# kolomeytsev/EB-CADRL

Measured on AMD Instinct MI355X. Metric: agent-steps/sec, higher is better.
Workload: dtype f64; 1 GPU; metric: 4096 envs/GPU x 10 humans + 8 static rows, ORCA + kinematics + collisions + reward + rotated obs (T=17), one ebc_step (one HIP launch) per step, auto-reset; envs_per_gpu=4096, humans=10, parallelism=env-slice x1

## Files before the change

### eb-cadrl_amd/csrc/ebc_kernels.h

```cpp
#pragma once

#include "ebc_device.h"

#ifndef EBC_ENV_PRIO
#define EBC_ENV_PRIO 3
#endif
#ifndef EBC_ORCA_PRIO
#define EBC_ORCA_PRIO 1
#endif
#ifndef EBC_POLL_SLEEP
#define EBC_POLL_SLEEP 2
#endif
#include "ebc_orca_group.h"
#include "ebc_scene_gen.h"
#include "ebc_step_rules.h"

namespace ebc {

struct DevState {
  int E, N, S, G;
  int *n_humans;
  double *px, *py, *vx, *vy, *gx, *gy, *radius, *v_pref;
  uint8_t *type;
  int *n_static;
  double *spx, *spy, *sradius;
  int *grid_scene;
  double *robot;
  double *robot_n;
  double *time;
  double *arrival;
  uint8_t *done;
  double *hact;
  uint4 *vel;
  unsigned long long *env_done;
  unsigned *rows_loaded;
  unsigned *robot_ready;
  unsigned *fault;
  ScenePool pool;
  float4 *tile;
  float inv_time_horizon, inv_time_step, range_sq;
  unsigned n_magic, n_shift;
};

#ifndef EBC_SPIN_LIMIT
#define EBC_SPIN_LIMIT (1u << 22)
#endif

struct StepIO {
  const double *robot_action;
  double border[4];
  int has_border;
  int robot_policy;
  int auto_reset;
  double *reward;
  uint8_t *done;
  uint8_t *info;
  double *dmin;
  double *dist_to_goal;
  double *robot_action_out;
  double *human_action;
  double *ob;
  float *obs_rotated;
};

struct LookIO {
  const double *actions;
  int A;
  double border[4];
  int has_border;
  double *reward;
  uint8_t *done;
  uint8_t *info;
  double *dmin;
  double *next_ob;
  float *rows;
};

__device__ __forceinline__ void store_tile(const EbcParams &p, const DevState &s, size_t k, double px,
                                           double py, double vx, double vy, double gx, double gy,
                                           double rad, double vpref) {
  float prefx, prefy;
  orca_pref_velocity(px, py, gx, gy, prefx, prefy);
  s.tile[2 * k] = make_float4((float)px, (float)py, (float)vx, (float)vy);
  s.tile[2 * k + 1] = make_float4((float)(rad + 0.01 + p.orca_safety_space), (float)vpref, prefx, prefy);
}

__global__ __launch_bounds__(256) void pool_pref_kernel(DevState s, size_t first, size_t count) {
  const size_t q = (size_t)blockIdx.x * blockDim.x + threadIdx.x;
  if (q >= count) return;
  const size_t k = first + q;
  float prefx, prefy;
  orca_pref_velocity(s.pool.px[k], s.pool.py[k], s.pool.gx[k], s.pool.gy[k], prefx, prefy);
  s.pool.pref[k] = make_float2(prefx, prefy);
}

__global__ __launch_bounds__(256) void rehome_grid_kernel(DevState s, uint64_t *grid) {
  const int e = blockIdx.x;
// ... 178 lines not shown
  const float posx = (float)rb[0], posy = (float)rb[1], velx = (float)rb[2], vely = (float)rb[3];
  float radius = (float)(rb[4] + 0.01 + safety_space), maxSpeed = (float)rb[7];
  float prefx, prefy;
  orca_pref_velocity(rb[0], rb[1], rb[5], rb[6], prefx, prefy);
  float opx = 0, opy = 0, ovx = 0, ovy = 0, orad = 0;
  if (valid) {
    opx = (float)row.px;
    opy = (float)row.py;
    ovx = (float)row.vx;
    ovy = (float)row.vy;
    orad = (float)(row.radius + 0.01 + safety_space);
  }
  if (sim.rows && l.e_ok) {
    const bool rebuild = sim.rows[ee] != n + ns;
    const size_t q = ee * (size_t)(N + S) + j;
    if (rebuild) {
      if (valid) sim.radius[q] = orad;
      if (j == 0) {
        sim.self[ee] = make_float2(radius, maxSpeed);
        sim.rows[ee] = n + ns;
      }
    } else {
      if (valid) orad = sim.radius[q];
      const float2 me = sim.self[ee];
      radius = me.x;
      maxSpeed = me.y;
    }
  }
  before_solve();
  orca_group<GS>(p, j, group, valid, posx, posy, velx, vely, radius, maxSpeed, prefx, prefy, opx, opy, ovx, ovy,
                 orad, dist_lds + group * L::Sh::DIST, lines_lds + group * L::Sh::LINES,
                 segs_lds + group * L::Sh::LINES, proj_lds + group * L::Sh::LINES, N + S, s.range_sq,
                 s.inv_time_horizon, s.inv_time_step, ox, oy);
}

template <int GS>
__global__ __launch_bounds__(EBC_WAVE) void orca_robot_kernel(EbcParams p, DevState s, double safety_space, double *act, RobotSim sim) {
  __shared__ __align__(16) unsigned char scratch[OrcaLds<GS>::BYTES];
  const RobotLane l = robot_lane<GS>(s);
  const ObsRow row = obs_row(env_rows(s, l.ee), l.j, l.n, l.ns);
  float ox, oy;
  orca_robot_solve<GS>(p, s, safety_space, sim, scratch, l, s.robot + l.ee * 9, row, ox, oy);
  if (l.e_ok && l.j == 0) {
    act[2 * l.ee] = (double)ox;
    act[2 * l.ee + 1] = (double)oy;
  }
}

template <typename Tp>
__device__ __forceinline__ void pin(Tp &x) {
  asm volatile("" : "+v"(x));
}

template <typename Tp>
__device__ __forceinline__ const Tp &read_late(const Tp &x) {
  typedef const Tp __attribute__((address_space(3))) *LdsPtr;
  unsigned off = (unsigned)(size_t)(LdsPtr)&x;
  asm volatile("" : "+v"(off));
  return *(const Tp *)(LdsPtr)(size_t)off;
}

struct ArgBlock {
  EbcParams p;
  DevState s;
  StepIO io;
};
template <typename Tp>
__device__ __forceinline__ void stage_args(Tp *dst_lds, const Tp &src, int lane) {
  const uint32_t *from = reinterpret_cast<const uint32_t *>(&src);
  uint32_t *to = reinterpret_cast<uint32_t *>(dst_lds);
  for (int w = lane; w < (int)(sizeof(Tp) / 4); w += EBC_WAVE) to[w] = from[w];
}

struct LaneMap {
  int el, i, n, ns;
  size_t ee, k;
  bool env_ok, active, leader;
};
struct HumanRegs {
  double px, py, vx, vy, gx, gy, rad, vpref, arrival;
  int type;
};

__device__ __forceinline__ LaneMap lane_map(const DevState &s, int e0, int epb, int lane) {
  LaneMap m;
  const int N = s.N;
  m.el = lane / N;
  m.i = lane - m.el * N;
  const int e = e0 + m.el;
  m.env_ok = m.el < epb && e < s.E;
  m.ee = m.env_ok ? (size_t)e : 0;
  m.k = m.ee * N + m.i;
  m.n = m.env_ok ? s.n_humans[m.ee] : 0;
  m.ns = (m.env_ok && s.S) ? s.n_static[m.ee] : 0;
  m.active = m.env_ok && m.i < m.n;
  m.leader = m.env_ok && m.i == 0;
  return m;
}

__device__ __forceinline__ HumanRegs load_human(const DevState &s, const LaneMap &m) {
  HumanRegs h = {0, 0, 0, 0, 0, 0, 0, 0, 0, 0};
  if (m.env_ok) {
    h.px = s.px[m.k];
    h.py = s.py[m.k];
    h.vx = s.vx[m.k];
    h.vy = s.vy[m.k];
    h.gx = s.gx[m.k];
    h.gy = s.gy[m.k];
    h.rad = s.radius[m.k];
    h.vpref = s.v_pref[m.k];
    h.type = s.type[m.k];
    h.arrival = s.arrival[m.k];
  }
  return h;
}

#define EBC_MAXT 4
struct CommitPre {
  int cursor;
  double sx[EBC_MAXT], sy[EBC_MAXT], sr[EBC_MAXT];
  double px, py, vx, vy, gx, gy, rad, vpref, spx, spy, srad, robot[9];
  int type, n_humans, n_static;
};

template <bool WITH_ROBOT = true>
__device__ __forceinline__ CommitPre preload_commit(const DevState &s, const StepIO &io, const LaneMap &m) {
  CommitPre c;
#pragma unroll
  for (int t = 0; t < EBC_MAXT; ++t) {
    const int r = m.i + t * s.N;
    const bool st = m.env_ok && (io.ob || io.obs_rotated) && r >= m.n && r - m.n < m.ns;
    const size_t q = m.ee * s.S + (st ? r - m.n : 0);
    c.sx[t] = st ? s.spx[q] : 0.0;
    c.sy[t] = st ? s.spy[q] : 0.0;
    c.sr[t] = st ? s.sradius[q] : 0.0;
  }
  c.cursor = 0;
  c.px = c.py = c.vx = c.vy = c.gx = c.gy = c.rad = c.vpref = c.spx = c.spy = c.srad = 0;
  c.type = c.n_humans = c.n_static = 0;
#pragma unroll
  for (int q = 0; q < 9; ++q) c.robot[q] = 0;
  if (io.auto_reset && m.env_ok) {
    const ScenePool &P = s.pool;
    c.cursor = P.P > 0 ? P.cursor[m.ee] : (int)m.ee;
    const size_t src = (size_t)c.cursor * s.N + m.i;
    c.n_humans = P.n_humans[c.cursor];
    c.px = P.px[src]; c.py = P.py[src]; c.vx = P.vx[src]; c.vy = P.vy[src];
    c.gx = P.gx[src]; c.gy = P.gy[src]; c.rad = P.radius[src]; c.vpref = P.v_pref[src];
    c.type = P.type[src];
    if (s.S) {
      c.n_static = P.n_static[c.cursor];
      if (m.i < s.S) {
        const size_t q = (size_t)c.cursor * s.S + m.i;
        c.spx = P.spx[q]; c.spy = P.spy[q]; c.srad = P.sradius[q];
      }
    }
    if (WITH_ROBOT && m.leader) {
#pragma unroll
      for (int q = 0; q < 9; ++q) c.robot[q] = P.robot[(size_t)c.cursor * 9 + q];
    }
  }
  return c;
}

__device__ __forceinline__ void pin_loads(HumanRegs &h, CommitPre &c, double (&rb)[9], double &gtime) {
  pin(h.px); pin(h.py); pin(h.vx); pin(h.vy); pin(h.gx); pin(h.gy); pin(h.rad); pin(h.vpref);
  pin(h.arrival); pin(h.type);
  pin(c.cursor);
#pragma unroll
  for (int q = 0; q < 9; ++q) pin(rb[q]);
#pragma unroll
  for (int t = 0; t < EBC_MAXT; ++t) { pin(c.sx[t]); pin(c.sy[t]); pin(c.sr[t]); }
  pin(gtime);
// ... 288 lines not shown
    h.px = h.px + ax * dt;
    h.py = h.py + ay * dt;
    h.vx = ax;
    h.vy = ay;
    if (h.arrival == 0 && norm2(h.px - h.gx, h.py - h.gy) < h.rad) h.arrival = tnew;
  } else {
    ax = 0;
    ay = 0;
  }
  const RotFrame f = rot_frame(rbn, p.rotate_unicycle);
  pin_pool(pre);
  if (m.leader && !restore) {
#pragma unroll
    for (int c = 0; c < 9; ++c) A.robot[c] = rbn[c];
    *A.time = tnew;
  }
  if (A.human_action) {
    A.human_action[0] = ax;
    A.human_action[1] = ay;
  }
  if (io.ob || io.obs_rotated) {
    int t = 0;
    for (int r = m.i; r < R; r += N, ++t) {
      double opx = 0, opy = 0, ovx = 0, ovy = 0, orad = 0;
      int otype = 0;
      bool valid = false;
      if (r < m.n) {
        opx = h.px; opy = h.py; ovx = h.vx; ovy = h.vy; orad = h.rad; otype = h.type;
        valid = true;
      } else if (r - m.n < m.ns) {
        if (t < EBC_MAXT) {
          opx = t == 0 ? pre.sx[0] : t == 1 ? pre.sx[1] : t == 2 ? pre.sx[2] : pre.sx[3];
          opy = t == 0 ? pre.sy[0] : t == 1 ? pre.sy[1] : t == 2 ? pre.sy[2] : pre.sy[3];
          orad = t == 0 ? pre.sr[0] : t == 1 ? pre.sr[1] : t == 2 ? pre.sr[2] : pre.sr[3];
        } else {
          const size_t q = m.ee * S + (r - m.n);
          opx = s.spx[q]; opy = s.spy[q]; orad = s.sradius[q];
        }
        otype = EBC_ADULT_STATIC;
        valid = true;
      }
      if (A.ob) {
        double *o = A.ob + (size_t)r * 5;
        o[0] = opx; o[1] = opy; o[2] = ovx; o[3] = ovy; o[4] = orad;
      }
      if (A.obs) {
        float out[T];
        if (valid) {
          rotate_row<T>(f, opx, opy, ovx, ovy, orad, otype, out);
        } else {
#pragma unroll
          for (int c = 0; c < T; ++c) out[c] = 0.0f;
        }
        float *o = A.obs + (m.ee * R + r) * T;
#pragma unroll
        for (int c = 0; c < T; ++c) o[c] = out[c];
      }
    }
  }
  commit_state_tail(p, s, m, h, pre, A, restore);
}

__device__ __forceinline__ void load_robot(const DevState &s, const LaneMap &m, double rb[9]) {
  const double *rb_in = s.robot + m.ee * 9;
#pragma unroll
  for (int c = 0; c < 9; ++c) rb[c] = m.env_ok ? rb_in[c] : 0.0;
}

template <int POLICY, int T>
__global__ __launch_bounds__(EBC_WAVE) void step_kernel(EbcParams p_in, DevState s_in, StepIO io_in) {
  const WaveTrace wt(1);
  const int lane = threadIdx.x;
  __shared__ ArgBlock args;
  __shared__ EnvScratch env_scratch;
  __shared__ double sh_rbn[EBC_WAVE][9];
  stage_args(&args.p, p_in, lane);
  stage_args(&args.s, s_in, lane);
  stage_args(&args.io, io_in, lane);
  wave_sync();
  const EbcParams &p = args.p;
  const DevState &s = args.s;
  const StepIO &io = args.io;
  const int epb = EBC_WAVE / s.N;
  const LaneMap m = lane_map(s, blockIdx.x * epb, epb, lane);
  double rb[9];
  load_robot(s, m, rb);
  double gtime = m.env_ok ? s.time[m.ee] : 0.0;
  HumanRegs h = load_human(s, m);
  CommitPre pre = preload_commit(s, io, m);
  const CommitAddr A = commit_addr(s, io, m);
  double ax = 0, ay = 0;
  if (POLICY == EBC_HUMAN_LINEAR) {
    if (m.active) linear_policy(h.px, h.py, h.gx, h.gy, h.vpref, ax, ay);
  } else if (m.env_ok) {
    ax = s.hact[m.k * 2];
    ay = s.hact[m.k * 2 + 1];
  }
  pin_loads(h, pre, rb, gtime);
  pin(ax);
  pin(ay);
  int done_flag = service_env(p, s, io, m, h, rb, gtime, lane, env_scratch);
  if (m.leader) {
#pragma unroll
    for (int c = 0; c < 9; ++c) sh_rbn[m.el][c] = rb[c];
  }
  done_flag = __shfl(done_flag, lane - m.i, EBC_WAVE);
  wave_sync();
  if (!m.env_ok) return;
  double rbn[9];
#pragma unroll
  for (int c = 0; c < 9; ++c) rbn[c] = sh_rbn[m.el][c];
  service_commit<T>(p, s, io, m, h, pre, A, rbn, io.auto_reset && done_flag, gtime + p.time_step, ax, ay);
}

struct StepGrid {
  unsigned env_blocks, orca_blocks, rows_blocks;
  unsigned rows_epw;
  unsigned epoch;
  unsigned total;
};

#define EBC_RBN_ENVS 16
struct RoleLds {
  ArgBlock args;
  union {
    double restart_robot[EBC_RBN_ENVS][9];
    EnvScratch env;
  };
};

#define EBC_ENV_LANES 4
__device__ __forceinline__ void env_lane_role(const EbcParams &p_in, const DevState &s_in, const StepIO &io_in, RoleLds &L,
                                              unsigned block, unsigned epoch, int lane) {
  stage_args(&L.args.p, p_in, lane);
  stage_args(&L.args.s, s_in, lane);
  stage_args(&L.args.io, io_in, lane);
  wave_sync();
  const EbcParams &p = L.args.p;
  const DevState &s = L.args.s;
  const StepIO &io = L.args.io;
  constexpr int Q = EBC_ENV_LANES, EPW = EBC_WAVE / Q;
  const int el = lane / Q, part = lane - el * Q;
  const int e0 = (int)block * EPW;
  const int e = e0 + el;
  const bool ok = e < s.E;
  const size_t ee = ok ? (size_t)e : 0;
  const int N = s.N;
  double rb[9];
#pragma unroll
  for (int c = 0; c < 9; ++c) rb[c] = ok ? s.robot[ee * 9 + c] : 0.0;
  const int n = ok ? s.n_humans[ee] : 0;
  double gtime = ok ? s.time[ee] : 0.0;
  int grid_slot = (ok && s.pool.grid) ? s.grid_scene[ee] : 0;
  const int chunk = (N + Q - 1) / Q;
  const int i0 = part * chunk;
  pin(gtime); pin(grid_slot);
#pragma unroll
  for (int c = 0; c < 9; ++c) pin(rb[c]);
  double a0 = 0, a1 = 0;
  if (ok) robot_action(io.robot_policy, io.robot_action, ee, rb, a0, a1);
  EBC_MARK(1);
  {
    double rn[9];
#pragma unroll
    for (int c = 0; c < 9; ++c) rn[c] = rb[c];
    robot_advance(p, rn, a0, a1);
    double *stage = &L.env.cand[0][0];
    if (part == 0) {
#pragma unroll
      for (int c = 0; c < 9; ++c) stage[el * 9 + c] = rn[c];
      L.env.gtime[el] = gtime;
      L.env.slot[el] = grid_slot;
      L.env.goal[el][0] = rb[5];
      L.env.goal[el][1] = rb[6];
      L.env.ract[el][0] = rn[0];
      L.env.ract[el][1] = rn[1];
    }
    wave_sync();
    const int here = min(EPW, s.E - e0);
    for (int q = lane; q < 9 * here; q += EBC_WAVE)
      __hip_atomic_store(s.robot_n + (size_t)e0 * 9 + q, stage[q], __ATOMIC_RELAXED, __HIP_MEMORY_SCOPE_AGENT);
  }
  constexpr int PRE = 2;
  double hpx[PRE], hpy[PRE], hvx[PRE], hvy[PRE], hr[PRE];
  int ht[PRE];
  {
    const DevState &sl = read_late(s);
#pragma unroll
    for (int q = 0; q < PRE; ++q) {
      const int i = i0 + q;
      const bool have = ok && q < chunk && i < N;
      const size_t k = ee * N + (have ? i : 0);
      hpx[q] = have ? sl.px[k] : 0.0; hpy[q] = have ? sl.py[k] : 0.0; hvx[q] = have ? sl.vx[k] : 0.0; hvy[q] = have ? sl.vy[k] : 0.0;
      hr[q] = have ? sl.radius[k] : 0.0;
      ht[q] = have ? (int)sl.type[k] : 0;
    }
  }
  double rvx, rvy;
  if (p.robot_kinematics == EBC_HOLONOMIC) {
    rvx = a0;
    rvy = a1;
  } else {
    rvx = a0 * cos(a1 + rb[8]);
    rvy = a0 * sin(a1 + rb[8]);
  }
  double dmin[3] = {INFINITY, INFINITY, INFINITY};
  int coll[4] = {0, 0, 0, 0};
  auto visit = [&](double px, double py, double vx, double vy, double r, int t) {
    const double d = closest_dist(px, py, vx, vy, r, rb[0], rb[1], rb[4], rvx, rvy, p.time_step);
#pragma unroll
    for (int q = 0; q < 3; ++q) {
      if (t == q && !coll[q]) {
        if (d < 0) coll[q] = 1;
        else if (d < dmin[q]) dmin[q] = d;
      }
    }
  };
#pragma unroll
  for (int q = 0; q < PRE; ++q)
    if (q < chunk && i0 + q < n) visit(hpx[q], hpy[q], hvx[q], hvy[q], hr[q], ht[q]);
  for (int q = PRE; q < chunk; ++q) {
    const int i = i0 + q;
    if (!__any(i < n)) break;
    if (i < n) {
      const size_t k = ee * N + i;
      visit(s.px[k], s.py[k], s.vx[k], s.vy[k], s.radius[k], (int)s.type[k]);
    }
  }
  asm volatile("s_waitcnt vmcnt(0)" ::: "memory");
  if (ok && part == 0) mailbox_put(s.robot_ready + ee, epoch);
  double fm[3] = {INFINITY, INFINITY, INFINITY};
  int fc[3] = {0, 0, 0};
  const int base = lane - part;
#pragma unroll
  for (int src = 0; src < Q; ++src) {
#pragma unroll
    for (int t = 0; t < 3; ++t) {
      const double od = __shfl(dmin[t], base + src, EBC_WAVE);
      const int oc = __shfl(coll[t], base + src, EBC_WAVE);
      if (!fc[t]) {
        fm[t] = od < fm[t] ? od : fm[t];
        fc[t] = oc;
      }
    }
  }
  EBC_MARK(2);
  if (ok && part == 0) {
    const EnvScratch &XL = read_late(L.env);
    const double nx = XL.ract[el][0], ny = XL.ract[el][1];
    int c4[4] = {fc[0], fc[1], fc[2], 0};
    c4[3] = grid_collision(s.pool.grid ? s.pool.grid + (size_t)XL.slot[el] * s.G * 2 : nullptr, s.G, p.map_size_m,
                           p.map_resolution, nx, ny, rb[4], io.has_border ? io.border : nullptr);
    EBC_MARK(3);
    const RewardOut ro = reward_compute(p, nx, ny, XL.goal[el][0], XL.goal[el][1], rb[4], a1, XL.gtime[el], fm, c4);
    s.done[ee] = (uint8_t)ro.done;
    if (io.reward) io.reward[ee] = ro.reward;
    if (io.done) io.done[ee] = (uint8_t)ro.done;
    if (io.info) io.info[ee] = (uint8_t)ro.info;
    if (io.dmin) {
      io.dmin[3 * ee] = fm[0];
      io.dmin[3 * ee + 1] = fm[1];
      io.dmin[3 * ee + 2] = fm[2];
    }
    if (io.dist_to_goal) io.dist_to_goal[ee] = ro.dist_to_goal;
    if (io.robot_action_out) {
      io.robot_action_out[2 * ee] = a0;
      io.robot_action_out[2 * ee + 1] = a1;
    }
    mailbox_put(s.env_done + ee, ((unsigned long long)epoch << 32) | (1u + (unsigned)ro.done));
  }
  EBC_MARK(4);
}

template <typename Tp>
__device__ __forceinline__ void sreg(const Tp &x) {
  asm volatile("" ::"s"(x));
}

template <int GS>
__device__ __forceinline__ void orca_role(const EbcParams &p, const DevState &s, const OrcaHot &hot, uint4 *vel, unsigned epoch,
                                          unsigned char *scratch, unsigned block, int lane) {
  sreg(s.robot); sreg(s.range_sq); sreg(s.inv_time_horizon); sreg(s.inv_time_step);
  sreg(p.robot_visible); sreg(p.orca_max_neighbors); sreg(p.orca_safety_space);
  constexpr int HPW = EBC_WAVE / GS;
  const int group = lane / GS, j = lane - group * GS;
  const unsigned hh = block * HPW + group;
  const bool h_ok = group < HPW && hh < (unsigned)hot.E * (unsigned)hot.N;
  int e, i;
  split_human(hot, hh, h_ok, e, i);
  float ox, oy;
  bool human_ok;
  orca_wave<GS>(p, s, hot, h_ok, e, i, scratch, ox, oy, human_ok);
#ifdef EBC_WAVE_TRACE
  if (h_ok && (int)hh == g_withhold_human) return;
#endif
  if (h_ok && j == 0) {
    const u32x4 w = {human_ok ? __float_as_uint(ox) : 0u, epoch, human_ok ? __float_as_uint(oy) : 0u, epoch};
    store16_device(vel + hh, w);
  }
}

template <int T>
__device__ __forceinline__ void rows_role(const EbcParams &p_in, const DevState &s_in, const StepIO &io_in,
                                          RoleLds &L, unsigned block, unsigned epw, unsigned epoch, int lane) {
  stage_args(&L.args.p, p_in, lane);
  stage_args(&L.args.s, s_in, lane);
  stage_args(&L.args.io, io_in, lane);
  wave_sync();
  const EbcParams &p = L.args.p;
  const DevState &s = L.args.s;
  const StepIO &io = L.args.io;
  const int N = s.N, S = s.S, R = N + S;
  const int el = R <= EBC_WAVE ? lane / R : 0;
  const int first = lane - el * R;
  const int e = (int)(block * epw) + el;
  const bool env_ok = el < (int)epw && e < s.E;
  const size_t ee = env_ok ? (size_t)e : 0;
  const int stride = R <= EBC_WAVE ? R : EBC_WAVE;
  RotFrame f = {};
  int n = env_ok ? s.n_humans[ee] : 0;
  int ns = (env_ok && S) ? s.n_static[ee] : 0;
  for (int slot = first; slot < R; slot += stride) {
    const bool human = slot < N;
    const size_t k = ee * N + (human ? slot : 0), q = ee * (size_t)(S ? S : 1) + (human ? 0 : slot - N);
    double opx = 0, opy = 0, ovx = 0, ovy = 0, orad = 0;
    int otype = 0;
    if (env_ok && human) {
      opx = s.px[k]; opy = s.py[k]; orad = s.radius[k]; otype = s.type[k];
    } else if (env_ok) {
      opx = s.spx[q]; opy = s.spy[q]; orad = s.sradius[q]; otype = EBC_ADULT_STATIC;
    }
    const uint4 *vbox = s.vel + k;
    pin(opx); pin(opy); pin(orad); pin(otype); pin(vbox); pin(n); pin(ns);
    if (slot == first) {
      mailbox_wait_epoch(s.robot_ready + ee, env_ok, epoch, s.fault);
      double rb[9];
#pragma unroll
      for (int c = 0; c < 9; ++c)
        rb[c] = env_ok ? __hip_atomic_load(s.robot_n + ee * 9 + c, __ATOMIC_RELAXED, __HIP_MEMORY_SCOPE_AGENT) : 0.0;
      f = rot_frame(rb, p.rotate_unicycle);
      pin(f.px); pin(f.py); pin(f.dg);
    }
    if (env_ok && slot + stride >= R && first == 0) mailbox_put(s.rows_loaded + ee, epoch);
    const bool valid = human ? slot < n : slot - N < ns;
    const int row = human ? (valid ? slot : ns + slot) : (valid ? n + slot - N : slot);
    auto emit = [&]() {
      if (!valid) opx = opy = ovx = ovy = orad = 0.0;
      if (io.ob) {
        double *o = io.ob + (ee * R + row) * 5;
        o[0] = opx; o[1] = opy; o[2] = ovx; o[3] = ovy; o[4] = orad;
      }
      if (io.obs_rotated) {
        float out[T];
        if (valid) {
          rotate_row<T>(f, opx, opy, ovx, ovy, orad, otype, out);
        } else {
#pragma unroll
          for (int c = 0; c < T; ++c) out[c] = 0.0f;
        }
        float *o = io.obs_rotated + (ee * R + row) * T;
#pragma unroll
        for (int c = 0; c < T; ++c) __builtin_nontemporal_store(out[c], o + c);
      }
    };
    const bool moving = human && valid;
    if (env_ok && !moving) emit();
    const u32x4 v = velocity_wait(vbox, env_ok && human, epoch, s.fault);
    if (env_ok && moving) {
      double ax, ay;
      unpack_velocity(v, ax, ay);
      opx = opx + ax * p.time_step;
      opy = opy + ay * p.time_step;
      ovx = ax;
      ovy = ay;
      emit();
    }
  }
}

__device__ __forceinline__ void state_role(const EbcParams &p_in, const DevState &s_in, const StepIO &io_in,
                                           RoleLds &L, int block, bool wait_rows, unsigned epoch, int lane) {
  stage_args(&L.args.p, p_in, lane);
  stage_args(&L.args.s, s_in, lane);
  stage_args(&L.args.io, io_in, lane);
  wave_sync();
  const EbcParams &p = L.args.p;
  const DevState &s = L.args.s;
  const StepIO &io = L.args.io;
  const int epb = EBC_WAVE / s.N;
  const LaneMap m = lane_map(s, block * epb, epb, lane);
  double gtime = m.env_ok ? s.time[m.ee] : 0.0;
  HumanRegs h = load_human(s, m);
  StepIO io_state = io;
  io_state.ob = nullptr;
  io_state.obs_rotated = nullptr;
  const uint4 *vbox = s.vel + m.k;
  unsigned long long *done_box = s.env_done + m.ee;
  unsigned *loaded_box = s.rows_loaded + m.ee;
  CommitPre pre = preload_commit<false>(s, io_state, m);
  float rprefx = 0, rprefy = 0;
  const bool parked = m.el < EBC_RBN_ENVS;
  if (io.auto_reset && m.env_ok) {
    const float2 rp = s.pool.pref[(size_t)pre.cursor * s.N + m.i];
    rprefx = rp.x;
    rprefy = rp.y;
    if (m.leader && parked) {
      const double *src = s.pool.robot + (size_t)pre.cursor * 9;
#pragma unroll
      for (int q = 0; q < 9; ++q) L.restart_robot[m.el][q] = src[q];
    }
  }
  const float tile_rad = (float)(h.rad + 0.01 + p.orca_safety_space), tile_max = (float)h.vpref;
  pin(vbox); pin(done_box); pin(loaded_box);
  pin(h.px); pin(h.py); pin(h.gx); pin(h.gy); pin(h.rad); pin(h.arrival); pin(gtime);
  pin(pre.cursor); pin(pre.px); pin(pre.py); pin(pre.vx); pin(pre.vy); pin(pre.gx); pin(pre.gy); pin(pre.rad);
  pin(pre.vpref); pin(pre.spx); pin(pre.spy); pin(pre.srad); pin(pre.type); pin(pre.n_humans); pin(pre.n_static);
  pin(rprefx); pin(rprefy);
  wave_sync();
  EBC_MARK(0);
  u32x4 v = {0u, 0u, 0u, 0u};
  unsigned d = 0;
  {
    bool wv = m.env_ok, wd = m.env_ok, wr = m.env_ok && wait_rows;
    for (unsigned spins = 0;; ++spins) {
      unsigned long long dw = 0;
      unsigned r = epoch;
      if (wd) dw = __hip_atomic_load(done_box, __ATOMIC_RELAXED, __HIP_MEMORY_SCOPE_AGENT);
      if (wr) r = __hip_atomic_load(loaded_box, __ATOMIC_RELAXED, __HIP_MEMORY_SCOPE_AGENT);
      if (wv) v = load16_device(vbox);
      wv = wv && (v.y != epoch || v.w != epoch);
      if (wd && (unsigned)(dw >> 32) == epoch) {
        d = (unsigned)dw;
        wd = false;
      }
      wr = wr && r != epoch;
      if (!__any(wv || wd || wr)) break;
      if (spins > EBC_SPIN_LIMIT) {
        if (wv || wd || wr) atomicOr(s.fault, 1u);
        break;
      }
      __builtin_amdgcn_s_sleep(EBC_POLL_SLEEP);
    }
  }
  EBC_MARK(1);
  if (!m.env_ok) return;
  const bool restore = io.auto_reset && d == 2u;
  const double tnew = gtime + p.time_step;
  const int N = s.N, S = s.S;
  float4 *tile = s.tile + 2 * m.k;
  double ax = 0, ay = 0;
  if (m.active) unpack_velocity(v, ax, ay);
  if (io.human_action) {
    io.human_action[m.k * 2] = ax;
    io.human_action[m.k * 2 + 1] = ay;
  }
  if (!restore) {
    if (m.active) {
      h.px = h.px + ax * p.time_step;
      h.py = h.py + ay * p.time_step;
      const double dx = h.gx - h.px, dy = h.gy - h.py;
      const double dist = norm2(dx, dy);
      const bool arrived_now = h.arrival == 0 && dist < h.rad;
      if (arrived_now) h.arrival = tnew;
      float prefx, prefy;
      orca_pref_from(dx, dy, dist, prefx, prefy);
      typedef float v4f __attribute__((ext_vector_type(4)));
      const v4f t0 = {(float)h.px, (float)h.py, (float)ax, (float)ay}, t1 = {tile_rad, tile_max, prefx, prefy};
      __builtin_nontemporal_store(h.px, s.px + m.k);
      __builtin_nontemporal_store(h.py, s.py + m.k);
      __builtin_nontemporal_store(ax, s.vx + m.k);
      __builtin_nontemporal_store(ay, s.vy + m.k);
      if (arrived_now) __builtin_nontemporal_store(h.arrival, s.arrival + m.k);
      __builtin_nontemporal_store(t0, reinterpret_cast<v4f *>(tile));
      __builtin_nontemporal_store(t1, reinterpret_cast<v4f *>(tile + 1));
    }
    if (m.leader) s.time[m.ee] = tnew;
  } else {
    const ScenePool &P = s.pool;
    const bool live = m.i < pre.n_humans;
    s.px[m.k] = live ? pre.px : 0.0;
    s.py[m.k] = live ? pre.py : 0.0;
    s.vx[m.k] = live ? pre.vx : 0.0;
    s.vy[m.k] = live ? pre.vy : 0.0;
    s.arrival[m.k] = 0.0;
    s.gx[m.k] = live ? pre.gx : 0.0;
    s.gy[m.k] = live ? pre.gy : 0.0;
    s.radius[m.k] = live ? pre.rad : 0.0;
    s.v_pref[m.k] = live ? pre.vpref : 0.0;
    s.type[m.k] = live ? (uint8_t)pre.type : (uint8_t)0;
    if (live) {
      tile[0] = make_float4((float)pre.px, (float)pre.py, (float)pre.vx, (float)pre.vy);
      tile[1] = make_float4((float)(pre.rad + 0.01 + p.orca_safety_space), (float)pre.vpref, rprefx, rprefy);
    } else {
      tile[0] = make_float4(0, 0, 0, 0);
      tile[1] = make_float4(0, 0, 0, 0);
    }
    if (m.i < S) {
      s.spx[m.ee * S + m.i] = pre.spx;
      s.spy[m.ee * S + m.i] = pre.spy;
      s.sradius[m.ee * S + m.i] = pre.srad;
    }
    for (int q = m.i + N; q < S; q += N) {
      const size_t c = (size_t)pre.cursor * S + q;
      s.spx[m.ee * S + q] = P.spx[c];
      s.spy[m.ee * S + q] = P.spy[c];
      s.sradius[m.ee * S + q] = P.sradius[c];
    }
    if (m.leader) {
      s.n_humans[m.ee] = pre.n_humans;
      if (S) s.n_static[m.ee] = pre.n_static;
      s.grid_scene[m.ee] = pre.cursor;
      double *rdst = s.robot_n + m.ee * 9;
      if (parked) {
#pragma unroll
        for (int q = 0; q < 9; ++q) rdst[q] = L.restart_robot[m.el][q];
      } else {
        const double *src = P.robot + (size_t)pre.cursor * 9;
        for (int q = 0; q < 9; ++q) rdst[q] = src[q];
      }
      s.time[m.ee] = 0.0;
      if (P.P > 0) {
        int nxt = pre.cursor - s.E + P.stride;
        P.cursor[m.ee] = s.E + (nxt >= P.P ? nxt % P.P : nxt);
      }
    }
  }
  EBC_MARK(2);
}

#ifndef EBC_STEP_WAVES
#define EBC_STEP_WAVES(GS) ((GS) <= 9 ? 6 : 5)
#endif
#ifndef EBC_STEP_WPB
#define EBC_STEP_WPB 1
#endif
template <int GS, int T>
__global__ __launch_bounds__(EBC_WAVE * EBC_STEP_WPB, EBC_STEP_WAVES(GS)) void orca_step_kernel(
    unsigned env_blocks, unsigned orca_blocks, int hot_E, int hot_N, unsigned hot_magic, unsigned hot_shift,
    const float4 *hot_tile, const int *hot_n_humans, uint4 *hot_vel, unsigned hot_epoch, unsigned pad,
    EbcParams p_in, DevState s_in, StepIO io_in, StepGrid g) {
  const WaveTrace wt(2);
  constexpr size_t LDS = ((sizeof(RoleLds) > (size_t)OrcaLds<GS>::BYTES ? sizeof(RoleLds) : (size_t)OrcaLds<GS>::BYTES) + 15) / 16 * 16;
  __shared__ __align__(16) unsigned char lds_all[EBC_STEP_WPB][LDS];
  unsigned char *lds = lds_all[threadIdx.x / EBC_WAVE];
  RoleLds &L = *reinterpret_cast<RoleLds *>(lds);
  const int lane = threadIdx.x & (EBC_WAVE - 1);
  unsigned b = blockIdx.x * EBC_STEP_WPB + threadIdx.x / EBC_WAVE;
  if (EBC_STEP_WPB > 1 && b >= g.total) return;
  if (b < env_blocks) {
    __builtin_amdgcn_s_setprio(EBC_ENV_PRIO);
    env_lane_role(p_in, s_in, io_in, L, b, g.epoch, lane);
    return;
  }
  b -= env_blocks;
  if (b < orca_blocks) {
    __builtin_amdgcn_s_setprio(EBC_ORCA_PRIO);
    const OrcaHot hot{hot_E, hot_N, hot_magic, hot_shift, hot_tile, hot_n_humans};
    orca_role<GS>(p_in, s_in, hot, hot_vel, hot_epoch, lds, b, lane);
    return;
  }
  b -= orca_blocks;
  if (b < g.rows_blocks) {
    rows_role<T>(p_in, s_in, io_in, L, b, g.rows_epw, g.epoch, lane);
    return;
  }
  b -= g.rows_blocks;
  state_role(p_in, s_in, io_in, L, (int)b, g.rows_blocks != 0, g.epoch, lane);
}

__global__ __launch_bounds__(64) void scene_gen_kernel(EbcSceneGen c, const uint32_t *seeds, uint32_t seed0, int n, int N, int S,
                                                        int G, SceneRow d, uint32_t *mt, int *status) {
  const int r = blockIdx.x * blockDim.x + threadIdx.x;
  if (r >= n) return;
  const size_t k = (size_t)r * N, q = (size_t)r * (S ? S : 1);
  const SceneRow o = {d.n_humans + r, d.px + k, d.py + k, d.vx + k, d.vy + k, d.gx + k, d.gy + k, d.radius + k, d.v_pref + k,
                      d.type + k, d.n_static + r, d.spx + q, d.spy + q, d.sradius + q,
                      d.grid ? d.grid + (size_t)r * G * 2 : nullptr, d.robot + (size_t)r * 9,
                      d.poly ? d.poly + q * 8 : nullptr, d.n_poly ? d.n_poly + r : nullptr};
  const int st = generate_scene_row(c, seeds ? seeds[r] : seed0 + (uint32_t)r, mt + r, (size_t)n, o, N, S, G);
  if (st) atomicOr(status, st);
}

__global__ __launch_bounds__(256) void il_targets_kernel(const double *reward, const uint8_t *done, const uint8_t *info, int K,
                                                         int E, double gamma_bar, double *values, uint8_t *keep) {
  const int e = blockIdx.x * blockDim.x + threadIdx.x;
  if (e >= E) return;
  double run = 0.0;
  uint8_t closed = 0;
  for (int t = K - 1; t >= 0; --t) {
    const size_t q = (size_t)t * E + e;
    const double r = reward[q];
    if (done[q]) {
      const uint8_t c = info[q];
      run = r;
      closed = (c == EBC_INFO_REACH_GOAL || c == EBC_INFO_COLLISION_OBSTACLE || c == EBC_INFO_COLLISION_ADULT ||
                c == EBC_INFO_COLLISION_BICYCLE || c == EBC_INFO_COLLISION_CHILD) ? 1 : 0;
    } else {
      run = r + gamma_bar * run;
    }
    values[q] = run;
    keep[q] = closed;
  }
}

__global__ __launch_bounds__(256) void row_counts_kernel(DevState s, long long *out) {
  const int e = blockIdx.x * blockDim.x + threadIdx.x;
  if (e < s.E) out[e] = (long long)s.n_humans[e] + (s.S ? s.n_static[e] : 0);
}

template <int T>
__global__ __launch_bounds__(256) void observe_kernel(EbcParams p, DevState s, double *ob, float *obs) {
  const int R = s.N + s.S;
  const size_t g = (size_t)blockIdx.x * blockDim.x + threadIdx.x;
  if (g >= (size_t)s.E * R) return;
  const size_t e = g / R;
  const int r = (int)(g - e * R);
  const int n = s.n_humans[e];
  const int ns = s.S ? s.n_static[e] : 0;
  const ObsRow row = obs_row(env_rows(s, e), r, n, ns);
  if (ob) {
    double *o = ob + g * 5;
    o[0] = row.px; o[1] = row.py; o[2] = row.vx; o[3] = row.vy; o[4] = row.radius;
  }
  if (obs) {
    float out[T];
    RotFrame f = {};
    if (row.valid) f = rot_frame(s.robot + e * 9, p.rotate_unicycle);
    rotated_row_or_zeros<T>(f, row, out);
    float *o = obs + g * T;
#pragma unroll
    for (int c = 0; c < T; ++c) o[c] = out[c];
  }
}

#define EBC_LA_THREADS 256
#define EBC_LA_MAX_ROWS 128
#define EBC_LA_MAX_ACTIONS 128
template <int POLICY, int T>
__global__ __launch_bounds__(EBC_LA_THREADS) void lookahead_kernel(EbcParams p, DevState s, LookIO io) {
  extern __shared__ __align__(16) unsigned char la_lds[];
  __shared__ double hpx[EBC_WAVE], hpy[EBC_WAVE], hvx[EBC_WAVE], hvy[EBC_WAVE], hrad[EBC_WAVE];
  __shared__ uint8_t htype[EBC_WAVE];
  __shared__ double row[EBC_LA_MAX_ROWS][5];
  __shared__ uint8_t row_type[EBC_LA_MAX_ROWS];
  __shared__ RotFrame frames[EBC_LA_MAX_ACTIONS];
  const int N = s.N, S = s.S, R = N + S, A = io.A;
  const int tid = threadIdx.x;
  const int e = blockIdx.x;
  const int n = s.n_humans[e];
  const int ns = S ? s.n_static[e] : 0;
// ... 132 lines not shown
```

### eb-cadrl_amd/csrc/ebc_trace.h

```cpp
#pragma once

#include <hip/hip_runtime.h>

namespace ebc {

#define EBC_TRACE_ROW 16

#ifdef EBC_WAVE_TRACE
__device__ unsigned long long *g_wave_trace;
__device__ unsigned g_wave_trace_blocks;
__device__ int g_withhold_human = -1;
__device__ __forceinline__ unsigned long long *wave_trace_row(int tag) {
  if (!g_wave_trace || blockIdx.x >= g_wave_trace_blocks) return nullptr;
  return g_wave_trace + ((size_t)tag * g_wave_trace_blocks + blockIdx.x) * EBC_TRACE_ROW;
}
__device__ __forceinline__ unsigned *wave_trace_lds() {
  __shared__ unsigned box[16];
  return box;
}
__device__ __forceinline__ bool wave_first_lane() {
  return (int)(threadIdx.x & 63) == __ffsll((long long)__ballot(1)) - 1;
}
__device__ __forceinline__ void wave_mark(int k) {
  const unsigned c = (unsigned)__builtin_amdgcn_s_memtime();
  if (wave_first_lane()) wave_trace_lds()[k] = c;
}
__device__ __forceinline__ void wave_count(int k) {
  if (wave_first_lane()) wave_trace_lds()[8 + k] += 1;
}
struct WaveTrace {
  int tag;
  __device__ __forceinline__ explicit WaveTrace(int t) : tag(t) {
#if EBC_WAVE_TRACE > 1
    if (threadIdx.x < 16) wave_trace_lds()[threadIdx.x] = 0;
#endif
    const unsigned long long r0 = __builtin_amdgcn_s_memrealtime(), c0 = __builtin_amdgcn_s_memtime();
    unsigned long long *o = wave_trace_row(t);
    if (o && threadIdx.x == 0) {
      o[0] = r0;
      o[2] = c0;
    }
  }
  __device__ __forceinline__ ~WaveTrace() {
    const unsigned long long r1 = __builtin_amdgcn_s_memrealtime(), c1 = __builtin_amdgcn_s_memtime();
    unsigned long long *o = wave_trace_row(tag);
    if (o && threadIdx.x == 0) {
      o[1] = r1;
      o[3] = c1;
#if EBC_WAVE_TRACE > 1
      o[4] = __builtin_amdgcn_s_getreg((4 << 0) | (0 << 6) | (31 << 11));
      const unsigned *box = wave_trace_lds();
      const unsigned c0 = (unsigned)o[2];
      for (int k = 0; k < 6; ++k) o[5 + k] = box[k] ? o[2] + (unsigned)(box[k] - c0) : 0;
      const unsigned long long prev_lp3 = o[12];
      for (int k = 0; k < 4; ++k) o[11 + k] = box[8 + k];
      o[15] = prev_lp3;
#endif
    }
  }
};
#if EBC_WAVE_TRACE > 1
#define EBC_MARK(k) ::ebc::wave_mark(k)
#define EBC_COUNT(k) ::ebc::wave_count(k)
#else
#define EBC_MARK(k)
#define EBC_COUNT(k)
#endif
#else
struct WaveTrace {
  __device__ __forceinline__ explicit WaveTrace(int) {}
};
#define EBC_MARK(k)
#define EBC_COUNT(k)
#endif

}
```

### eb-cadrl_amd/csrc/ebcsim.hip

```cpp
#include <hip/hip_runtime.h>

#include <cmath>
#include <cstdio>
#include <cstdlib>
#include <cstring>
#include <string>
#include <type_traits>
#include <utility>
#include <vector>

#include "ebc_host.h"
#include "ebc_dagger.h"
#include "ebc_kernels.h"
#include "ebc_local_map_kernel.h"
#include "ebc_rollout.h"
#include "ebc_sail_api.h"

namespace {

using ebc::DevState;
using ebc::LookIO;
using ebc::StepIO;

using ebc_host::fail;
// ... 100 lines not shown
    return EBC_OK;
  }
  int finish() {
    for (auto &o : outs)
      HIP_TRY(hipMemcpyAsync(o.host, o.dev, o.bytes, hipMemcpyDeviceToHost, h->stream));
    unsigned fault = 0;
    HIP_TRY(hipMemcpyAsync(&fault, h->s.fault, sizeof(fault), hipMemcpyDeviceToHost, h->stream));
    HIP_TRY(hipStreamSynchronize(h->stream));
    return report_fault(h, fault);
  }
};

size_t pad256(size_t b) { return (b + 255) & ~(size_t)255; }

int check_handle(void *handle, Handle **out) {
  if (!handle) return fail(EBC_ERR_INVALID, "null handle");
  *out = (Handle *)handle;
  hipError_t e = hipSetDevice((*out)->device);
  if (e != hipSuccess) return fail(EBC_ERR_DEVICE, std::string("hipSetDevice: ") + hipGetErrorString(e));
  return EBC_OK;
}

int orca_blocks(const Handle *h) {
  const long humans = (long)h->s.E * h->s.N;
  const int hpw = EBC_WAVE / h->orca_gs;
  return (int)((humans + hpw - 1) / hpw);
}

const int kGroupSizes[] = {2, 3, 4, 5, 6, 7, 8, 9, 10, 12, 16, 21, 32};

int group_size_for(int n) {
  for (int g : kGroupSizes)
    if (g >= n) return g;
  return 32;
}

#ifdef EBC_DEV_GS
constexpr int kDevHumanGs = EBC_DEV_GS, kDevRobotGs = 21;
#else
constexpr int kDevHumanGs = 0, kDevRobotGs = 0;
#endif

template <int DEV_GS, typename F>
int with_group_size(int gs, F f) {
  if constexpr (DEV_GS != 0) {
    if (gs != DEV_GS) return fail(EBC_ERR_UNSUPPORTED, "development build: " + std::to_string(DEV_GS) + "-lane ORCA groups only");
    return f(std::integral_constant<int, DEV_GS>());
  } else {
    switch (gs) {
#define GS_(N) case N: return f(std::integral_constant<int, N>())
      GS_(2); GS_(3); GS_(4); GS_(5); GS_(6); GS_(7); GS_(8); GS_(9); GS_(10); GS_(12); GS_(16); GS_(21);
#undef GS_
      default: return f(std::integral_constant<int, 32>());
    }
  }
}

int launch_orca(Handle *h) {
  const int blocks = orca_blocks(h);
  return with_group_size<kDevHumanGs>(h->orca_gs, [&](auto gs) -> int {
    hipLaunchKernelGGL((ebc::orca_kernel<decltype(gs)::value>), dim3(blocks), dim3(EBC_WAVE), 0, h->stream, h->p, h->s);
    HIP_TRY(hipGetLastError());
    return EBC_OK;
  });
}

template <int POLICY>
int launch_service(Handle *h, const StepIO &io) {
  const int epb = EBC_WAVE / h->s.N;
  const int blocks = (h->s.E + epb - 1) / epb;
  if (h->T == 17)
    hipLaunchKernelGGL((ebc::step_kernel<POLICY, 17>), dim3(blocks), dim3(EBC_WAVE), 0, h->stream, h->p, h->s, io);
  else
    hipLaunchKernelGGL((ebc::step_kernel<POLICY, 13>), dim3(blocks), dim3(EBC_WAVE), 0, h->stream, h->p, h->s, io);
  HIP_TRY(hipGetLastError());
  return EBC_OK;
}

template <int GS>
int launch_orca_step_gs(Handle *h, const StepIO &io, unsigned blocks, const ebc::StepGrid &g) {
  if (h->T == 17)
    hipLaunchKernelGGL((ebc::orca_step_kernel<GS, 17>), dim3((blocks + EBC_STEP_WPB - 1) / EBC_STEP_WPB), dim3(EBC_WAVE * EBC_STEP_WPB), 0, h->stream,
                       g.env_blocks, g.orca_blocks, h->s.E, h->s.N, h->s.n_magic, h->s.n_shift, (const float4 *)h->s.tile,
                       (const int *)h->s.n_humans, h->s.vel, g.epoch, 0u, h->p, h->s, io, g);
  else
    hipLaunchKernelGGL((ebc::orca_step_kernel<GS, 13>), dim3((blocks + EBC_STEP_WPB - 1) / EBC_STEP_WPB), dim3(EBC_WAVE * EBC_STEP_WPB), 0, h->stream,
                       g.env_blocks, g.orca_blocks, h->s.E, h->s.N, h->s.n_magic, h->s.n_shift, (const float4 *)h->s.tile,
                       (const int *)h->s.n_humans, h->s.vel, g.epoch, 0u, h->p, h->s, io, g);
  HIP_TRY(hipGetLastError());
  return EBC_OK;
}

int launch_orca_step(Handle *h, const StepIO &io) {
  const int epb = EBC_WAVE / h->s.N;
  const int R = h->s.N + h->s.S;
  ebc::StepGrid g;
  const unsigned state_blocks = (unsigned)((h->s.E + epb - 1) / epb);
  constexpr int envs_per_env_wave = EBC_WAVE / EBC_ENV_LANES;
  g.env_blocks = (unsigned)((h->s.E + envs_per_env_wave - 1) / envs_per_env_wave);
  g.orca_blocks = (unsigned)orca_blocks(h);
  g.rows_epw = R <= EBC_WAVE ? (unsigned)(EBC_WAVE / R) : 1u;
  g.rows_blocks = (io.ob || io.obs_rotated) ? (unsigned)((h->s.E + g.rows_epw - 1) / g.rows_epw) : 0u;
  const unsigned long long blocks = (unsigned long long)g.env_blocks + state_blocks + g.orca_blocks + g.rows_blocks;
  if (blocks >= 2147483648ull) return fail(EBC_ERR_UNSUPPORTED, "ORCA step grid >= 2^31 workgroups");
  if (++h->epoch == 0) h->epoch = 1;
  g.epoch = h->epoch;
  g.total = (unsigned)blocks;
  const int rc = with_group_size<kDevHumanGs>(
      h->orca_gs, [&](auto gs) { return launch_orca_step_gs<decltype(gs)::value>(h, io, (unsigned)blocks, g); });
  if (rc == EBC_OK) std::swap(h->s.robot, h->s.robot_n);
  return rc;
}

int launch_step(Handle *h, const StepIO &io, int policy) {
  if (policy == EBC_HUMAN_ORCA) return launch_orca_step(h, io);
  if (policy == EBC_HUMAN_LINEAR) return launch_service<EBC_HUMAN_LINEAR>(h, io);
  return launch_service<EBC_HUMAN_EXTERNAL>(h, io);
}

template <int POLICY>
int launch_lookahead(Handle *h, const LookIO &io) {
  const size_t lds = (size_t)io.A * h->s.N * 8 + (io.rows ? (size_t)EBC_LA_THREADS * h->T * 4 : 0);
  if (h->T == 17)
    hipLaunchKernelGGL((ebc::lookahead_kernel<POLICY, 17>), dim3(h->s.E), dim3(EBC_LA_THREADS), lds, h->stream, h->p, h->s, io);
  else
    hipLaunchKernelGGL((ebc::lookahead_kernel<POLICY, 13>), dim3(h->s.E), dim3(EBC_LA_THREADS), lds, h->stream, h->p, h->s, io);
  HIP_TRY(hipGetLastError());
  return EBC_OK;
}

struct SceneDst {
  int *n_humans;
  double *px, *py, *vx, *vy, *gx, *gy, *radius, *v_pref;
  uint8_t *type;
  int *n_static;
  double *spx, *spy, *sradius;
  uint64_t *grid;
  double *robot;
};

int alloc_pool(Handle *h, int P) {
  ebc::ScenePool old = h->s.pool;
  std::vector<void *> old_allocs = h->pool_allocs;
  uint64_t *old_grid = h->pool_grid_alloc;
  h->pool_allocs.clear();
  ebc::ScenePool &pl = h->s.pool;
  const int E = h->s.E;
  const size_t slots = (size_t)E + P;
  const size_t PN = slots * h->s.N, PS = slots * (h->s.S ? h->s.S : 1);
  const size_t EN = (size_t)E * h->s.N, ES = (size_t)E * (h->s.S ? h->s.S : 1);
  const bool keep = !old_allocs.empty();
  auto get = [&](auto **out, size_t count, const void *from, size_t keep_count) -> int {
    void *ptr = nullptr;
    const size_t bytes = count * sizeof(**out) + 16;
    HIP_TRY(hipMalloc(&ptr, bytes));
    HIP_TRY(hipMemset(ptr, 0, bytes));
    if (keep && from) HIP_TRY(hipMemcpy(ptr, from, keep_count * sizeof(**out), hipMemcpyDeviceToDevice));
    h->pool_allocs.push_back(ptr);
    *out = reinterpret_cast<std::remove_reference_t<decltype(*out)>>(ptr);
    return EBC_OK;
  };
  int rc = EBC_OK;
#define G_(f, c, k) if (rc == EBC_OK) rc = get(&pl.f, (c), old.f, (k))
  G_(n_humans, slots, E); G_(px, PN, EN); G_(py, PN, EN); G_(vx, PN, EN); G_(vy, PN, EN); G_(gx, PN, EN);
  G_(gy, PN, EN); G_(radius, PN, EN); G_(v_pref, PN, EN); G_(type, PN, EN); G_(n_static, slots, E);
  G_(spx, PS, ES); G_(spy, PS, ES); G_(sradius, PS, ES); G_(robot, slots * 9, (size_t)E * 9);
  G_(pref, PN, EN);
#undef G_
  if (rc == EBC_OK) rc = get(&h->pool_grid_alloc, slots * h->s.G * 2, old_grid, (size_t)E * h->s.G * 2);
  pl.grid = (keep && old.grid) ? h->pool_grid_alloc : nullptr;
  pl.P = P;
  pl.stride = 0;
  pl.cursor = old.cursor;
  for (void *ptr : old_allocs) (void)hipFree(ptr);
  return rc;
}

int upload_scene(Handle *h, const EbcScene *sc, const int32_t *ids, const SceneDst &d, bool with_grid,
                 hipMemcpyKind kind = hipMemcpyHostToDevice) {
  const int n = sc->n, N = h->s.N, S = h->s.S, G = h->s.G;
  bool contiguous = true;
  if (ids)
    for (int r = 0; r < n; ++r)
      if (ids[r] != ids[0] + r) contiguous = false;
  auto up = [&](void *dst_base, const void *src, size_t row_bytes) -> int {
    if (!src) return EBC_OK;
    if (contiguous) {
// ... 1228 lines not shown
```

Measured before the change: 2.515 billion agent-steps/s.

## Interleave step-kernel role blocks across eight env classes

Splits the environment range into eight contiguous classes and maps each role's block index round-robin across them (block r goes to class r%8, offset r/8), for ENV, ORCA, rows and state roles. Consecutive workgroups therefore touch different env slices, which likely spreads dependent producer/consumer roles across XCDs or CUs and balances the dispatch order. It changes which blocks run concurrently and may add partially filled waves at class boundaries. A trace tweak also reads an extra hardware register.

```diff
diff --git a/eb-cadrl_amd/csrc/ebc_kernels.h b/eb-cadrl_amd/csrc/ebc_kernels.h
--- a/eb-cadrl_amd/csrc/ebc_kernels.h
+++ b/eb-cadrl_amd/csrc/ebc_kernels.h
@@ -13,6 +13,7 @@
 #endif
 #include "ebc_orca_group.h"
 #include "ebc_scene_gen.h"
+#include "ebc_step_grid.h"
 #include "ebc_step_rules.h"
 
 namespace ebc {
@@ -357,13 +358,13 @@
   int type;
 };
 
-__device__ __forceinline__ LaneMap lane_map(const DevState &s, int e0, int epb, int lane) {
+__device__ __forceinline__ LaneMap lane_map(const DevState &s, int e0, int e_end, int epb, int lane) {
   LaneMap m;
   const int N = s.N;
   m.el = lane / N;
   m.i = lane - m.el * N;
   const int e = e0 + m.el;
-  m.env_ok = m.el < epb && e < s.E;
+  m.env_ok = m.el < epb && e < e_end;
   m.ee = m.env_ok ? (size_t)e : 0;
   m.k = m.ee * N + m.i;
   m.n = m.env_ok ? s.n_humans[m.ee] : 0;
@@ -818,7 +819,7 @@
   const DevState &s = args.s;
   const StepIO &io = args.io;
   const int epb = EBC_WAVE / s.N;
-  const LaneMap m = lane_map(s, blockIdx.x * epb, epb, lane);
+  const LaneMap m = lane_map(s, blockIdx.x * epb, s.E, epb, lane);
   double rb[9];
   load_robot(s, m, rb);
   double gtime = m.env_ok ? s.time[m.ee] : 0.0;
@@ -854,7 +855,9 @@
   unsigned rows_epw;
   unsigned epoch;
   unsigned total;
+  unsigned ec;
 };
+static_assert(EBC_GRID_WAVE == EBC_WAVE, "ebc_step_grid.h: lanes of a wave");
 
 #define EBC_RBN_ENVS 16
 struct RoleLds {
@@ -866,8 +869,9 @@
 };
 
 #define EBC_ENV_LANES 4
+static_assert(EBC_GRID_ENV_EPW == EBC_WAVE / EBC_ENV_LANES, "ebc_step_grid.h: envs per ENV wave");
 __device__ __forceinline__ void env_lane_role(const EbcParams &p_in, const DevState &s_in, const StepIO &io_in, RoleLds &L,
-                                              unsigned block, unsigned epoch, int lane) {
+                                              unsigned block, unsigned ec, unsigned epoch, int lane) {
   stage_args(&L.args.p, p_in, lane);
   stage_args(&L.args.s, s_in, lane);
   stage_args(&L.args.io, io_in, lane);
@@ -877,9 +881,10 @@
   const StepIO &io = L.args.io;
   constexpr int Q = EBC_ENV_LANES, EPW = EBC_WAVE / Q;
   const int el = lane / Q, part = lane - el * Q;
-  const int e0 = (int)block * EPW;
+  const StepSpan span = step_span(block, ec, (unsigned)s.E, EPW);
+  const int e0 = (int)span.first, e_end = (int)span.end;
   const int e = e0 + el;
-  const bool ok = e < s.E;
+  const bool ok = e < e_end;
   const size_t ee = ok ? (size_t)e : 0;
   const int N = s.N;
   double rb[9];
@@ -913,7 +918,7 @@
       L.env.ract[el][1] = rn[1];
     }
     wave_sync();
-    const int here = min(EPW, s.E - e0);
+    const int here = e_end - e0;
     for (int q = lane; q < 9 * here; q += EBC_WAVE)
       __hip_atomic_store(s.robot_n + (size_t)e0 * 9 + q, stage[q], __ATOMIC_RELAXED, __HIP_MEMORY_SCOPE_AGENT);
   }
@@ -1015,13 +1020,14 @@
 
 template <int GS>
 __device__ __forceinline__ void orca_role(const EbcParams &p, const DevState &s, const OrcaHot &hot, uint4 *vel, unsigned epoch,
-                                          unsigned char *scratch, unsigned block, int lane) {
+                                          unsigned char *scratch, unsigned block, unsigned class_humans, int lane) {
   sreg(s.robot); sreg(s.range_sq); sreg(s.inv_time_horizon); sreg(s.inv_time_step);
   sreg(p.robot_visible); sreg(p.orca_max_neighbors); sreg(p.orca_safety_space);
   constexpr int HPW = EBC_WAVE / GS;
   const int group = lane / GS, j = lane - group * GS;
-  const unsigned hh = block * HPW + group;
-  const bool h_ok = group < HPW && hh < (unsigned)hot.E * (unsigned)hot.N;
+  const StepSpan span = step_span(block, class_humans, (unsigned)hot.E * (unsigned)hot.N, HPW);
+  const unsigned hh = span.first + group;
+  const bool h_ok = hh < span.end;
   int e, i;
   split_human(hot, hh, h_ok, e, i);
   float ox, oy;
@@ -1038,7 +1044,7 @@
 
 template <int T>
 __device__ __forceinline__ void rows_role(const EbcParams &p_in, const DevState &s_in, const StepIO &io_in,
-                                          RoleLds &L, unsigned block, unsigned epw, unsigned epoch, int lane) {
+                                          RoleLds &L, unsigned block, unsigned ec, unsigned epw, unsigned epoch, int lane) {
   stage_args(&L.args.p, p_in, lane);
   stage_args(&L.args.s, s_in, lane);
   stage_args(&L.args.io, io_in, lane);
@@ -1049,8 +1055,9 @@
   const int N = s.N, S = s.S, R = N + S;
   const int el = R <= EBC_WAVE ? lane / R : 0;
   const int first = lane - el * R;
-  const int e = (int)(block * epw) + el;
-  const bool env_ok = el < (int)epw && e < s.E;
+  const StepSpan span = step_span(block, ec, (unsigned)s.E, epw);
+  const int e = (int)span.first + el;
+  const bool env_ok = e < (int)span.end;
   const size_t ee = env_ok ? (size_t)e : 0;
   const int stride = R <= EBC_WAVE ? R : EBC_WAVE;
   RotFrame f = {};
@@ -1115,7 +1122,7 @@
 }
 
 __device__ __forceinline__ void state_role(const EbcParams &p_in, const DevState &s_in, const StepIO &io_in,
-                                           RoleLds &L, int block, bool wait_rows, unsigned epoch, int lane) {
+                                           RoleLds &L, unsigned block, unsigned ec, bool wait_rows, unsigned epoch, int lane) {
   stage_args(&L.args.p, p_in, lane);
   stage_args(&L.args.s, s_in, lane);
   stage_args(&L.args.io, io_in, lane);
@@ -1124,7 +1131,8 @@
   const DevState &s = L.args.s;
   const StepIO &io = L.args.io;
   const int epb = EBC_WAVE / s.N;
-  const LaneMap m = lane_map(s, block * epb, epb, lane);
+  const StepSpan span = step_span(block, ec, (unsigned)s.E, (unsigned)epb);
+  const LaneMap m = lane_map(s, (int)span.first, (int)span.end, epb, lane);
   double gtime = m.env_ok ? s.time[m.ee] : 0.0;
   HumanRegs h = load_human(s, m);
   StepIO io_state = io;
@@ -1273,7 +1281,7 @@
 template <int GS, int T>
 __global__ __launch_bounds__(EBC_WAVE * EBC_STEP_WPB, EBC_STEP_WAVES(GS)) void orca_step_kernel(
     unsigned env_blocks, unsigned orca_blocks, int hot_E, int hot_N, unsigned hot_magic, unsigned hot_shift,
-    const float4 *hot_tile, const int *hot_n_humans, uint4 *hot_vel, unsigned hot_epoch, unsigned pad,
+    const float4 *hot_tile, const int *hot_n_humans, uint4 *hot_vel, unsigned hot_epoch, unsigned hot_class_humans,
     EbcParams p_in, DevState s_in, StepIO io_in, StepGrid g) {
   const WaveTrace wt(2);
   constexpr size_t LDS = ((sizeof(RoleLds) > (size_t)OrcaLds<GS>::BYTES ? sizeof(RoleLds) : (size_t)OrcaLds<GS>::BYTES) + 15) / 16 * 16;
@@ -1285,23 +1293,23 @@
   if (EBC_STEP_WPB > 1 && b >= g.total) return;
   if (b < env_blocks) {
     __builtin_amdgcn_s_setprio(EBC_ENV_PRIO);
-    env_lane_role(p_in, s_in, io_in, L, b, g.epoch, lane);
+    env_lane_role(p_in, s_in, io_in, L, b, g.ec, g.epoch, lane);
     return;
   }
   b -= env_blocks;
   if (b < orca_blocks) {
     __builtin_amdgcn_s_setprio(EBC_ORCA_PRIO);
     const OrcaHot hot{hot_E, hot_N, hot_magic, hot_shift, hot_tile, hot_n_humans};
-    orca_role<GS>(p_in, s_in, hot, hot_vel, hot_epoch, lds, b, lane);
+    orca_role<GS>(p_in, s_in, hot, hot_vel, hot_epoch, lds, b, hot_class_humans, lane);
     return;
   }
   b -= orca_blocks;
   if (b < g.rows_blocks) {
-    rows_role<T>(p_in, s_in, io_in, L, b, g.rows_epw, g.epoch, lane);
+    rows_role<T>(p_in, s_in, io_in, L, b, g.ec, g.rows_epw, g.epoch, lane);
     return;
   }
   b -= g.rows_blocks;
-  state_role(p_in, s_in, io_in, L, (int)b, g.rows_blocks != 0, g.epoch, lane);
+  state_role(p_in, s_in, io_in, L, b, g.ec, g.rows_blocks != 0, g.epoch, lane);
 }
 
 __global__ __launch_bounds__(64) void scene_gen_kernel(EbcSceneGen c, const uint32_t *seeds, uint32_t seed0, int n, int N, int S,
diff --git a/eb-cadrl_amd/csrc/ebc_step_grid.h b/eb-cadrl_amd/csrc/ebc_step_grid.h
--- /dev/null
+++ b/eb-cadrl_amd/csrc/ebc_step_grid.h
@@ -0,0 +1,52 @@
+#pragma once
+
+#define EBC_GRID_CLASSES 8
+#define EBC_GRID_WAVE 64
+#define EBC_GRID_ENV_EPW 16
+
+namespace ebc {
+
+struct StepSpan {
+  unsigned first, end;
+};
+
+constexpr StepSpan step_span(unsigned r, unsigned per_class, unsigned total, unsigned upw) {
+  const unsigned c = r % EBC_GRID_CLASSES, q = r / EBC_GRID_CLASSES;
+  const unsigned lo = c * per_class;
+  const unsigned class_end = lo + per_class < total ? lo + per_class : total;
+  const unsigned first = lo + q * upw;
+  const unsigned end = first + upw < class_end ? first + upw : class_end;
+  return StepSpan{first, end};
+}
+
+struct StepGridShape {
+  unsigned ec;
+  unsigned orca_hpw, rows_epw, state_epw;
+  unsigned long long env_blocks, orca_blocks, rows_blocks, state_blocks;
+
+  constexpr unsigned long long total() const { return env_blocks + orca_blocks + rows_blocks + state_blocks; }
+  constexpr bool fits() const { return total() < 2147483648ull; }
+  constexpr unsigned long long orca_base() const { return env_blocks; }
+  constexpr unsigned long long rows_base() const { return env_blocks + orca_blocks; }
+  constexpr unsigned long long state_base() const { return env_blocks + orca_blocks + rows_blocks; }
+};
+
+constexpr unsigned long long step_grid_role_blocks(unsigned long long per_class, unsigned upw) {
+  return EBC_GRID_CLASSES * ((per_class + upw - 1) / upw);
+}
+
+constexpr StepGridShape step_grid_shape(int E, int N, int S, int gs, bool rows) {
+  StepGridShape g{};
+  const int R = N + S;
+  g.ec = ((unsigned)E + EBC_GRID_CLASSES - 1) / EBC_GRID_CLASSES;
+  g.orca_hpw = (unsigned)(EBC_GRID_WAVE / gs);
+  g.rows_epw = R <= EBC_GRID_WAVE ? (unsigned)(EBC_GRID_WAVE / R) : 1u;
+  g.state_epw = (unsigned)(EBC_GRID_WAVE / N);
+  g.env_blocks = step_grid_role_blocks(g.ec, EBC_GRID_ENV_EPW);
+  g.orca_blocks = step_grid_role_blocks((unsigned long long)g.ec * (unsigned)N, g.orca_hpw);
+  g.rows_blocks = rows ? step_grid_role_blocks(g.ec, g.rows_epw) : 0ull;
+  g.state_blocks = step_grid_role_blocks(g.ec, g.state_epw);
+  return g;
+}
+
+}
diff --git a/eb-cadrl_amd/csrc/ebc_trace.h b/eb-cadrl_amd/csrc/ebc_trace.h
--- a/eb-cadrl_amd/csrc/ebc_trace.h
+++ b/eb-cadrl_amd/csrc/ebc_trace.h
@@ -48,7 +48,8 @@
       o[1] = r1;
       o[3] = c1;
 #if EBC_WAVE_TRACE > 1
-      o[4] = __builtin_amdgcn_s_getreg((4 << 0) | (0 << 6) | (31 << 11));
+      o[4] = (unsigned long long)__builtin_amdgcn_s_getreg((4 << 0) | (0 << 6) | (31 << 11)) |
+             (unsigned long long)__builtin_amdgcn_s_getreg((20 << 0) | (0 << 6) | (3 << 11)) << 32;
       const unsigned *box = wave_trace_lds();
       const unsigned c0 = (unsigned)o[2];
       for (int k = 0; k < 6; ++k) o[5 + k] = box[k] ? o[2] + (unsigned)(box[k] - c0) : 0;
diff --git a/eb-cadrl_amd/csrc/ebcsim.hip b/eb-cadrl_amd/csrc/ebcsim.hip
--- a/eb-cadrl_amd/csrc/ebcsim.hip
+++ b/eb-cadrl_amd/csrc/ebcsim.hip
@@ -206,27 +206,25 @@
   if (h->T == 17)
     hipLaunchKernelGGL((ebc::orca_step_kernel<GS, 17>), dim3((blocks + EBC_STEP_WPB - 1) / EBC_STEP_WPB), dim3(EBC_WAVE * EBC_STEP_WPB), 0, h->stream,
                        g.env_blocks, g.orca_blocks, h->s.E, h->s.N, h->s.n_magic, h->s.n_shift, (const float4 *)h->s.tile,
-                       (const int *)h->s.n_humans, h->s.vel, g.epoch, 0u, h->p, h->s, io, g);
+                       (const int *)h->s.n_humans, h->s.vel, g.epoch, g.ec * (unsigned)h->s.N, h->p, h->s, io, g);
   else
     hipLaunchKernelGGL((ebc::orca_step_kernel<GS, 13>), dim3((blocks + EBC_STEP_WPB - 1) / EBC_STEP_WPB), dim3(EBC_WAVE * EBC_STEP_WPB), 0, h->stream,
                        g.env_blocks, g.orca_blocks, h->s.E, h->s.N, h->s.n_magic, h->s.n_shift, (const float4 *)h->s.tile,
-                       (const int *)h->s.n_humans, h->s.vel, g.epoch, 0u, h->p, h->s, io, g);
+                       (const int *)h->s.n_humans, h->s.vel, g.epoch, g.ec * (unsigned)h->s.N, h->p, h->s, io, g);
   HIP_TRY(hipGetLastError());
   return EBC_OK;
 }
 
 int launch_orca_step(Handle *h, const StepIO &io) {
-  const int epb = EBC_WAVE / h->s.N;
-  const int R = h->s.N + h->s.S;
+  const ebc::StepGridShape shape = ebc::step_grid_shape(h->s.E, h->s.N, h->s.S, h->orca_gs, io.ob || io.obs_rotated);
+  if (!shape.fits()) return fail(EBC_ERR_UNSUPPORTED, "ORCA step grid >= 2^31 workgroups");
+  const unsigned long long blocks = shape.total();
   ebc::StepGrid g;
-  const unsigned state_blocks = (unsigned)((h->s.E + epb - 1) / epb);
-  constexpr int envs_per_env_wave = EBC_WAVE / EBC_ENV_LANES;
-  g.env_blocks = (unsigned)((h->s.E + envs_per_env_wave - 1) / envs_per_env_wave);
-  g.orca_blocks = (unsigned)orca_blocks(h);
-  g.rows_epw = R <= EBC_WAVE ? (unsigned)(EBC_WAVE / R) : 1u;
-  g.rows_blocks = (io.ob || io.obs_rotated) ? (unsigned)((h->s.E + g.rows_epw - 1) / g.rows_epw) : 0u;
-  const unsigned long long blocks = (unsigned long long)g.env_blocks + state_blocks + g.orca_blocks + g.rows_blocks;
-  if (blocks >= 2147483648ull) return fail(EBC_ERR_UNSUPPORTED, "ORCA step grid >= 2^31 workgroups");
+  g.env_blocks = (unsigned)shape.env_blocks;
+  g.orca_blocks = (unsigned)shape.orca_blocks;
+  g.rows_blocks = (unsigned)shape.rows_blocks;
+  g.rows_epw = shape.rows_epw;
+  g.ec = shape.ec;
   if (++h->epoch == 0) h->epoch = 1;
   g.epoch = h->epoch;
   g.total = (unsigned)blocks;
```

Result: faster. 2.541 billion agent-steps/s, median of 6 (+1.1%).
